# charles-cooper/Smoothed-Particle-Hydrodynamics

Hardware: AMD Instinct MI355X
Metric: particle-steps/sec (whole node) (higher is better)
Workload: dtype f32; 1 GPU; config4_16M_box; particles=16507704, particles_per_gpu=16507704, cell_ids=wide, parallelism=1 GPU

## Files before the change

smoothed-particle-hydrodynamics_amd/csrc/sph_neighbors.hip:

```cpp
#include <stdlib.h>
#include <string.h>

#include <mutex>

#include "sph_common.h"

__global__ __launch_bounds__(SPH_BLOCK) void k_clear_neighbors(int32_t* __restrict__ nbrId, float* __restrict__ nbrDist,
                                                                uint16_t* __restrict__ nbr16, size_t n4) {
  const size_t i = (size_t)blockIdx.x * SPH_BLOCK + threadIdx.x;
  if (i >= n4) return;
  reinterpret_cast<int4*>(nbrId)[i] = make_int4(-1, -1, -1, -1);
  reinterpret_cast<float4*>(nbrDist)[i] = make_float4(-1.f, -1.f, -1.f, -1.f);
  if (i < n4 / 2) reinterpret_cast<int4*>(nbr16)[i] = make_int4(-1, -1, -1, -1);
}

int sphk_clear_neighbors(sph_solver* s) {
  const size_t n4 = (size_t)((s->d.N + SPH_TILE - 1) / SPH_TILE) * 64 * 8;
  hipLaunchKernelGGL(k_clear_neighbors, dim3((unsigned)((n4 + SPH_BLOCK - 1) / SPH_BLOCK)), dim3(SPH_BLOCK), 0, s->stream,
                     s->d.nbrId, s->d.nbrDist, s->d.nbr16, n4);
  SPH_HIP(hipGetLastError());
  return SPH_OK;
}

struct FnParams {
  int G, gx, gy, rangeLo, rangeHi;
  int idxLo, idxHi;
  int gz, bandCap;
  float h, cellSize, cellSizeInv, simScale, xmin, ymin, zmin;
};
struct FnArrays {
  const float4* sortedPos;
  const uint32_t *keys, *cellStart;
  int32_t* nbrId;
  float* nbrDist;
  uint16_t* nbr16;
};

__device__ __forceinline__ int wrap_cell(int c, int G) {
  if (c < 0) c += G;
  if (c >= G) c -= G;
  return c;
}

#define FN_PART 128
#define FN_THREADS (2 * FN_PART)
#define FN_PER_WAVE 32
#define FN_WAVES (FN_THREADS / 64)
#define FN_CAND_CAP 4096
#define FN_STAGE_PER 8
#define FN_WIN 16
#define FN_CAND_PAD 16
#define FN_LIST_CAP 48
#define FN_CHUNK 8
#define FN_SLOTS_PER_LANE (SPH_MAXN / 2)

typedef float f32x2 __attribute__((ext_vector_type(2)));
typedef float f32x4 __attribute__((ext_vector_type(4)));

#define FN_DST_STRIDE 36
#define FN_STAGE_BYTES (FN_PER_WAVE * (FN_DST_STRIDE * 4 + SPH_MAXN * 2))
#define FN_LIST_ROWS ((FN_STAGE_BYTES + 127) / 128 > FN_LIST_CAP ? (FN_STAGE_BYTES + 127) / 128 : FN_LIST_CAP)

struct FnShared {
  float x[FN_CAND_CAP + FN_CAND_PAD], y[FN_CAND_CAP + FN_CAND_PAD], z[FN_CAND_CAP + FN_CAND_PAD];
  uint16_t list[FN_WAVES][FN_LIST_ROWS][64];
  float binU[64];
  int rowLo[9], rowHi[9], rowBase[9];
  int win[9][FN_WIN];
  int winTrue[9][FN_WIN];
  uint32_t hist[FN_WAVES][32];
#ifdef FN_STAMPS
  uint32_t stamps[16];
#endif
};
static_assert(FN_LIST_ROWS >= FN_LIST_CAP, "the wave's list area holds the lists first, the staging of the store phase afterwards");

__device__ __forceinline__ int pair_other(int v) { return __builtin_amdgcn_update_dpp(0, v, 0xB1, 0xf, 0xf, true); }
typedef unsigned long long fn_mask_t;
static_assert(FN_LIST_CAP <= 64, "one bit per list entry");

#ifdef FN_STAMPS
#define FN_STAMP(ph)                                                                                      \
  {                                                                                                       \
    const unsigned long long t_ = __builtin_amdgcn_s_memtime();                                           \
    if ((threadIdx.x & 63) == 0) atomicAdd(&sh.stamps[(ph)], (uint32_t)(t_ - stamp_));                    \
    stamp_ = __builtin_amdgcn_s_memtime();                                                                \
  }
#else
#define FN_STAMP(ph)
#endif

template <bool BANDS>
__device__ __forceinline__ void fn_exact_walk(const FnParams& d, const FnArrays& g, FnShared& sh, int id, int wave, int lane) {
  const float4 me = g.sortedPos[id];
  const int myCell = (int)g.keys[id];
  int lo[8], hi[8], ldsBase[8];
  {
    const float px = me.x - d.xmin, py = me.y - d.ymin, pz = me.z - d.zmin;
    const float cfx = (float)(int)(me.x * d.cellSizeInv) * d.cellSize;
    const float cfy = (float)(int)(me.y * d.cellSizeInv) * d.cellSize;
    const float cfz = (float)(int)(me.z * d.cellSizeInv) * d.cellSize;
    const int dx = ((px - cfx) < d.h) ? -1 : 1;
    const int dy = ((py - cfy) < d.h) ? -1 : 1;
    const int dz = ((pz - cfz) < d.h) ? -1 : 1;
    const int sy = dy * d.gx, sz = dz * d.gx * d.gy;
    const int off[8] = {0, dx, sy, sz, dx + sy, dx + sz, sy + sz, dx + sy + sz};
    const int ry = dy + 1, rz = dz + 1;
    const int rows[8] = {4, 4, ry + 3, 1 + 3 * rz, ry + 3, 1 + 3 * rz, ry + 3 * rz, ry + 3 * rz};
#pragma unroll
    for (int k = 0; k < 8; k++) {
      const int raw = myCell + off[k];
      int c = wrap_cell(raw, d.G);
      const int r = (c == raw && (!BANDS || rows[k] == 4)) ? rows[k] : -1;
      c = min(max(c, 0), d.G - 1);
      lo[k] = (int)g.cellStart[c];
      hi[k] = (int)g.cellStart[c + 1];
      if (hi[k] - lo[k] > (1 << 20)) hi[k] = lo[k];
      ldsBase[k] = -1;
      if (r >= 0 && hi[k] > lo[k] && lo[k] >= sh.rowLo[r] && hi[k] <= sh.rowHi[r]) ldsBase[k] = sh.rowBase[r] + (lo[k] - sh.rowLo[r]);
    }
  }
  if (lane < 32) sh.hist[wave][lane] = 0u;
  const unsigned long long ltMask = (lane == 0) ? 0ull : (~0ull >> (64 - lane));
  const float h2 = d.h * d.h;
#pragma unroll
  for (int k = 0; k < 8; k++) {
    for (int j0 = lo[k]; j0 < hi[k]; j0 += 64) {
      const int j = j0 + lane;
      if (j < hi[k] && j != id) {
        float ox, oy, oz;
        if (ldsBase[k] >= 0) { const int sl = ldsBase[k] + (j - lo[k]); ox = sh.x[sl]; oy = sh.y[sl]; oz = sh.z[sl]; }
        else { const float4 o = g.sortedPos[j]; ox = o.x; oy = o.y; oz = o.z; }
        const float ex = me.x - ox, ey = me.y - oy, ez = me.z - oz;
        const float d2 = ex * ex + ey * ey + ez * ez;
        if (d2 <= h2) {
          const float dist = sqrtf(d2);
          const int bin = (int)(dist * (float)SPH_RSEG / d.h);
          if (bin < SPH_RSEG) atomicAdd(&sh.hist[wave][bin], 1u);
        }
      }
    }
  }
  int jb = 0, sum = 0;
  while (jb < SPH_RSEG) {
    sum += (int)sh.hist[wave][jb];
    if (sum == SPH_MAXN) break;
    if (sum > SPH_MAXN) { jb--; break; }
    jb++;
  }
  const float r_thr = (float)(jb + 1) * d.h / (float)SPH_RSEG;
  const float r2 = r_thr * r_thr;
  int found = 0;
#pragma unroll
  for (int k = 0; k < 8; k++) {
    for (int j0 = lo[k]; j0 < hi[k] && found < SPH_MAXN; j0 += 64) {
      const int j = j0 + lane;
      float d2 = 0.f;
      bool hit = false;
      if (j < hi[k] && j != id) {
        float ox, oy, oz;
        if (ldsBase[k] >= 0) { const int sl = ldsBase[k] + (j - lo[k]); ox = sh.x[sl]; oy = sh.y[sl]; oz = sh.z[sl]; }
        else { const float4 o = g.sortedPos[j]; ox = o.x; oy = o.y; oz = o.z; }
        const float ex = me.x - ox, ey = me.y - oy, ez = me.z - oz;
        d2 = ex * ex + ey * ey + ez * ez;
        hit = d2 <= r2;
      }
      const unsigned long long m = __ballot(hit);
      const int pos = found + __popcll(m & ltMask);
      if (hit && pos < SPH_MAXN) {
        const size_t idx = nbr_index(id, pos);
        g.nbrId[idx] = j;
        g.nbrDist[idx] = sqrtf(d2) * d.simScale;
      }
      found += __popcll(m);
    }
  }
  if (lane >= min(found, SPH_MAXN) && lane < SPH_MAXN) {
    const size_t idx = nbr_index(id, lane);
    g.nbrId[idx] = -1;
    g.nbrDist[idx] = -1.f;
  }
  if (lane == 0) g.nbr16[nbr_index(id, 0)] = (uint16_t)SPH_N16_WIDE;
}

template <bool BANDS>
__global__ __launch_bounds__(FN_THREADS, 2) void k_find_neighbors(FnParams d, const float4* __restrict__ sortedPos,
                                                                   const uint32_t* __restrict__ keys,
                                                                   const uint32_t* __restrict__ cellStart,
                                                                   const float* __restrict__ binU, int32_t* __restrict__ nbrId,
                                                                   float* __restrict__ nbrDist, uint16_t* __restrict__ nbr16,
                                                                   int32_t* __restrict__ nbrBase, uint32_t* __restrict__ dbg,
                                                                   uint32_t* __restrict__ trace,
                                                                   const float4* __restrict__ bandPos,
                                                                   const uint32_t* __restrict__ bandStart) {
  extern __shared__ __align__(16) unsigned char fn_smem[];
  FnShared& sh = *reinterpret_cast<FnShared*>(fn_smem);
  const int tid = threadIdx.x, lane = tid & 63, wave = tid >> 6;
  const int p = tid >> 1, laneB = tid & 1;
  const int rangeBegin = max((int)cellStart[d.rangeLo], d.idxLo), rangeEnd = min((int)cellStart[d.rangeHi], d.idxHi);
  const int p0 = rangeBegin + blockIdx.x * FN_PART;
  if (p0 >= rangeEnd) return;
  const int id = p0 + p;
  const bool alive = id < rangeEnd;
  FnArrays g;
  g.sortedPos = sortedPos; g.keys = keys; g.cellStart = cellStart; g.nbrId = nbrId; g.nbrDist = nbrDist; g.nbr16 = nbr16;
#ifdef FN_STAMPS
  const unsigned long long wgStart_ = __builtin_amdgcn_s_memrealtime();
  if (tid < 16) sh.stamps[tid] = 0u;
  __syncthreads();
  unsigned long long stamp_ = __builtin_amdgcn_s_memtime();
#endif

  const int blockHi = min(p0 + FN_PART, rangeEnd);
  const float4 myPos = alive ? sortedPos[id] : make_float4(0.f, 0.f, 0.f, 0.f);
  const int myCell = alive ? (int)keys[id] : 0;
  int batchLo = p0, retry = 0;
  while (batchLo < blockHi) {
  int batchHi = blockHi;
  if (retry) {
    const unsigned row0 = keys[batchLo] / (unsigned)d.gx;
    int firstStop = FN_PART;
#pragma unroll
    for (int q = FN_PART / 64 - 1; q >= 0; q--) {
      const int iq = batchLo + 64 * q + lane;
      const bool stopq = (iq >= blockHi) || (keys[min(iq, blockHi - 1)] / (unsigned)d.gx != row0) || (retry == 2 && (q > 0 || lane >= 32));
      const unsigned long long mq = __ballot(stopq);
      if (mq) firstStop = 64 * q + __ffsll((long long)mq) - 1;
    }
    batchHi = min(batchLo + firstStop, blockHi);
  }
  const int cLo = (int)keys[batchLo], cHi = (int)keys[batchHi - 1];
  const int nc = cHi - cLo + 3;
  const bool winOk = nc + 1 <= FN_WIN;
  constexpr int order[9] = {4, 3, 5, 1, 7, 0, 2, 6, 8};
  int runLo[9], runN[9], total = 0;
  {
    const int q = min(lane >> 1, 8);
    const int r = (int)((0x862071534ull >> (4 * q)) & 15ull);
    const int shift = (r % 3 - 1) * d.gx + (r / 3 - 1) * d.gx * d.gy;
    const int cell = ((lane & 1) ? cHi + 2 : cLo - 1) + shift;
    const uint32_t* tbl = cellStart;
    if (BANDS && r != 4) tbl = bandStart + (size_t)(r - (r > 4 ? 1 : 0)) * ((size_t)d.G + 1);
    const int v = (int)tbl[min(max(cell, 0), d.G)];
#pragma unroll
    for (int qq = 0; qq < 9; qq++) {
      const int lo = __builtin_amdgcn_readlane(v, 2 * qq), hi = __builtin_amdgcn_readlane(v, 2 * qq + 1);
      runLo[qq] = lo; runN[qq] = max(hi - lo, 0);
      total += runN[qq];
    }
  }
  if (total > FN_CAND_CAP) {
    if (retry < 2) { retry++; continue; }
    total = 0;
#pragma unroll
    for (int q = 0; q < 9; q++) {
      if (total + runN[q] > FN_CAND_CAP) { runN[q] = 0; if (tid == 0) atomicAdd(&dbg[3], 1u); }
      total += runN[q];
    }
  }
  int se[9], sd[9];
  {
    int base = 0;
#pragma unroll
    for (int q = 0; q < 9; q++) { sd[q] = runLo[q] - base; base += runN[q]; se[q] = base; }
    if (BANDS) {
#pragma unroll
      for (int q = 1; q < 9; q++) sd[q] += (order[q] - (order[q] > 4 ? 1 : 0)) * d.bandCap;
    }
  }
  if (tid == 0) {
#pragma unroll
    for (int q = 0; q < 9; q++) { sh.rowLo[order[q]] = runLo[q]; sh.rowHi[order[q]] = runLo[q] + runN[q]; sh.rowBase[order[q]] = se[q] - runN[q]; }
  }
  if (winOk && tid < 9 * FN_WIN) {
    const int r = tid / FN_WIN, i = tid % FN_WIN;
    const int shift = (r % 3 - 1) * d.gx + (r / 3 - 1) * d.gx * d.gy;
    const int wc = min(max(cLo - 1 + shift + i, 0), d.G);
    if (BANDS) {
      const uint32_t* tbl = (r == 4) ? cellStart : bandStart + (size_t)(r - (r > 4 ? 1 : 0)) * ((size_t)d.G + 1);
      if (i <= nc) { sh.win[r][i] = (int)tbl[wc]; sh.winTrue[r][i] = (int)cellStart[wc]; }
    } else {
      if (i <= nc) sh.win[r][i] = (int)cellStart[wc];
    }
  }
  if (tid >= 192 && tid < 256) sh.binU[tid - 192] = binU[tid - 192];
  FN_STAMP(0)
  {
    constexpr int PER = FN_STAGE_PER;
#pragma unroll 1
    for (int f0 = 0; f0 < total; f0 += PER * FN_THREADS) {
      float4 rec[PER];
#pragma unroll
      for (int u = 0; u < PER; u++) {
        const int f = min(f0 + tid + u * FN_THREADS, total - 1);
        int delta = sd[0];
#pragma unroll
        for (int q = 0; q < 8; q++) delta = (f >= se[q]) ? sd[q + 1] : delta;
        if (BANDS) rec[u] = (f >= se[0] ? bandPos : sortedPos)[f + delta];
        else rec[u] = sortedPos[f + delta];
      }
#pragma unroll
      for (int u = 0; u < PER; u++) {
        const int f = f0 + tid + u * FN_THREADS;
        if (f < total) { sh.x[f] = rec[u].x; sh.y[f] = rec[u].y; sh.z[f] = rec[u].z; }
      }
    }
  }
  __syncthreads();
  FN_STAMP(3)
  const bool mine_now = alive && id >= batchLo && id < batchHi;
  bool slow = false;

  if (mine_now) {
  float4 me = myPos;
  int myCellNow = myCell, idNow = id;
  asm volatile("" : "+v"(me.x), "+v"(me.y), "+v"(me.z), "+v"(myCellNow), "+v"(idNow));
  int pLo[4], pHi[4], absDelta[4];
  int selfSlot = -1;
  int zLoMine = 0;
  int trueLo[4] = {0, 0, 0, 0}, trueHi[4] = {0, 0, 0, 0};
  {
    const float px = me.x - d.xmin, py = me.y - d.ymin, pz = me.z - d.zmin;
    const float cfx = (float)(int)(me.x * d.cellSizeInv) * d.cellSize;
    const float cfy = (float)(int)(me.y * d.cellSizeInv) * d.cellSize;
    const float cfz = (float)(int)(me.z * d.cellSizeInv) * d.cellSize;
    const int dx = ((px - cfx) < d.h) ? -1 : 1;
    const int dy = ((py - cfy) < d.h) ? -1 : 1;
    const int dz = ((pz - cfz) < d.h) ? -1 : 1;
    const int sy = dy * d.gx, sz = dz * d.gx * d.gy;
    const int ry = dy + 1, rz = dz + 1;
    const bool stepX[4] = {laneB != 0, laneB == 0, laneB == 0, laneB == 0};
    const bool stepY[4] = {false, true, false, true};
    const bool stepZ[4] = {false, false, true, true};
#pragma unroll
    for (int i = 0; i < 4; i++) {
      const int xs = stepX[i] ? dx : 0;
      const int raw = myCellNow + xs + (stepY[i] ? sy : 0) + (stepZ[i] ? sz : 0);
      const int row = (stepY[i] ? ry : 1) + 3 * (stepZ[i] ? rz : 1);
      const int c = wrap_cell(raw, d.G);
      int lo, hi;
      int tLo, tHi;
      const bool staged = c == raw;
      const bool banded = BANDS && i != 0;
      if (staged && winOk) {
        const int w = myCellNow - cLo + 1 + xs;
        lo = sh.win[row][w];
        hi = sh.win[row][w + 1];
        tLo = lo; tHi = hi;
        if (banded) { tLo = sh.winTrue[row][w]; tHi = sh.winTrue[row][w + 1]; }
      } else {
        const int cc = min(max(c, 0), d.G - 1);
        lo = tLo = (int)cellStart[cc];
        hi = tHi = (int)cellStart[cc + 1];
        if (banded && staged) {
          const uint32_t* tbl = bandStart + (size_t)(row - (row > 4 ? 1 : 0)) * ((size_t)d.G + 1);
          lo = (int)tbl[cc];
          hi = (int)tbl[cc + 1];
        }
      }
      const int n = hi - lo;
      int base = 0;
      if (n > 0) {
        if (staged && lo >= sh.rowLo[row] && hi <= sh.rowHi[row]) base = sh.rowBase[row] + (lo - sh.rowLo[row]);
        else slow = true;
      }
      pLo[i] = base;
      pHi[i] = base + n;
      absDelta[i] = lo - base;
      if (banded) absDelta[i] += (row - (row > 4 ? 1 : 0)) * d.bandCap;
      if (i == 2) zLoMine = tLo;
      if (i == 0 && laneB == 0) selfSlot = base + (idNow - lo);
      if (BANDS) { trueLo[i] = tLo; trueHi[i] = tHi; }
    }
    if (BANDS) {
      const int cx = (int)(me.x * d.cellSizeInv), cy = (int)(me.y * d.cellSizeInv), cz = (int)(me.z * d.cellSizeInv);
      const bool premise = me.x >= 0.f && me.y >= 0.f && me.z >= 0.f && me.x < 1.0e9f && me.y < 1.0e9f && me.z < 1.0e9f && cx < d.gx &&
                           cy < d.gy && cz < d.gz && myCellNow == cx + cy * d.gx + cz * d.gx * d.gy;
      if (!premise) slow = true;
    }
  }
  int wideB = 0;
  if (BANDS) {
    const int zOther = pair_other(zLoMine);
    const int zB = laneB ? zLoMine : zOther;
#pragma unroll
    for (int i = 0; i < 4; i++) {
      const bool zf = i >= 2;
      const int rel = SPH_N16_BIAS - (zf ? zB : idNow);
      if (trueHi[i] > trueLo[i] && (trueLo[i] + rel < 0 || trueHi[i] - 1 + rel > SPH_N16_MAX)) wideB = 1;
    }
  }
  {
    const int other = pair_other((int)slow);
    slow = slow || (other != 0);
  }
  if (slow) {
#pragma unroll
    for (int i = 0; i < 4; i++) pHi[i] = pLo[i];
    if (laneB == 0) atomicAdd(&dbg[0], 1u);
  }
  FN_STAMP(4)

  int cnt = 0;
  int segEnd[4];
  const f32x2 mx = {me.x, me.x}, my = {me.y, me.y}, mz = {me.z, me.z};
  const float r2f = sh.binU[63];
  const f32x2 nthr = {-r2f, -r2f};
  float neg1s = -1.f;
  asm volatile("" : "+s"(neg1s));
  const f32x2 neg1 = {neg1s, neg1s};
  uint16_t (*const myList)[64] = sh.list[wave];
#define FN_DIFF(m, c) __builtin_elementwise_fma((c), neg1, (m))
#define FN_TEST(X, Y, Z)                                                                        \
  {                                                                                             \
    const f32x2 ex0 = FN_DIFF(mx, X.xy), ex1 = FN_DIFF(mx, X.zw), ey0 = FN_DIFF(my, Y.xy), ey1 = FN_DIFF(my, Y.zw); \
    const f32x2 ez0 = FN_DIFF(mz, Z.xy), ez1 = FN_DIFF(mz, Z.zw);                               \
    const f32x2 s0 = __builtin_elementwise_fma(ez0, ez0, __builtin_elementwise_fma(ey0, ey0, __builtin_elementwise_fma(ex0, ex0, nthr))); \
    const f32x2 s1 = __builtin_elementwise_fma(ez1, ez1, __builtin_elementwise_fma(ey1, ey1, __builtin_elementwise_fma(ex1, ex1, nthr))); \
    acc = __builtin_amdgcn_alignbit(acc, __float_as_uint(s0.x), 31);                            \
    acc = __builtin_amdgcn_alignbit(acc, __float_as_uint(s0.y), 31);                            \
    acc = __builtin_amdgcn_alignbit(acc, __float_as_uint(s1.x), 31);                            \
    acc = __builtin_amdgcn_alignbit(acc, __float_as_uint(s1.y), 31);                            \
  }
#define FN_FLUSH(k)                                                                             \
  {                                                                                             \
    uint32_t m = ((k) == 0) ? 0u : (acc << (32 - (k)));          \
    const int lowT = pieceLo - aBase, hiT = pieceHi - aBase;                                    \
    if (lowT > 0) m &= 0xffffffffu >> lowT;                \
    if (hiT < 32) m &= ~(0xffffffffu >> hiT);                         \
    if (i == 0) {                                                      \
      const unsigned ts = (unsigned)(selfSlot - aBase);                                         \
      if (ts < 32u) m &= ~(0x80000000u >> ts);                                                  \
    }                                                                                           \
    cnt += __popc(m);                                                                           \
    if (cnt > FN_LIST_CAP) m = 0u;                         \
    while (m != 0u) {                                                                           \
      const int bpos = __clz((int)m);                                                           \
      *wr = (uint16_t)(aBase + bpos);                                                           \
      wr += 64;                                                    \
      m &= ~(0x80000000u >> bpos);                                                              \
    }                                                                                           \
  }
  uint16_t* wr = &myList[0][lane];
#pragma unroll
  for (int i = 0; i < 4; i++) {
    const int pieceLo = pLo[i], pieceHi = pHi[i];
    if (pieceHi > pieceLo) {
      int a = pieceLo & ~3;
      int aBase = a, k = 0;
      uint32_t acc = 0u;
      f32x4 X = *reinterpret_cast<const f32x4*>(&sh.x[a]);
      f32x4 Y = *reinterpret_cast<const f32x4*>(&sh.y[a]);
      f32x4 Z = *reinterpret_cast<const f32x4*>(&sh.z[a]);
      f32x4 Xb = *reinterpret_cast<const f32x4*>(&sh.x[a + 4]);
      f32x4 Yb = *reinterpret_cast<const f32x4*>(&sh.y[a + 4]);
      f32x4 Zb = *reinterpret_cast<const f32x4*>(&sh.z[a + 4]);
      while (a < pieceHi) {
        FN_TEST(X, Y, Z)
        X = *reinterpret_cast<const f32x4*>(&sh.x[a + 8]);
        Y = *reinterpret_cast<const f32x4*>(&sh.y[a + 8]);
        Z = *reinterpret_cast<const f32x4*>(&sh.z[a + 8]);
        __builtin_amdgcn_sched_barrier(0);
        FN_TEST(Xb, Yb, Zb)
        Xb = *reinterpret_cast<const f32x4*>(&sh.x[a + 12]);
        Yb = *reinterpret_cast<const f32x4*>(&sh.y[a + 12]);
        Zb = *reinterpret_cast<const f32x4*>(&sh.z[a + 12]);
        __builtin_amdgcn_sched_barrier(0);
        a += 8; k += 8;
        if (k == 32) { FN_FLUSH(32) aBase = a; k = 0; }
      }
      FN_FLUSH(k)
    }
    segEnd[i] = cnt;
  }
#undef FN_TEST
#undef FN_FLUSH
  FN_STAMP(5)
  int over = cnt > FN_LIST_CAP ? 1 : 0;
  over |= pair_other(over);
  if (over) {
    if (laneB == 0 && !slow) atomicAdd(&dbg[1], 1u);
    slow = true;
#pragma unroll
    for (int i = 0; i < 4; i++) segEnd[i] = 0;
  }

  const int total = segEnd[3];
  float d2v[FN_LIST_CAP];
  uint32_t slotPk[FN_LIST_CAP / 2];
  int idxv[FN_LIST_CAP];
#pragma unroll
  for (int c0 = 0; c0 < FN_LIST_CAP; c0 += FN_CHUNK) {
    if (__any(c0 < total)) {
      int slotv[FN_CHUNK];
#pragma unroll
      for (int u = 0; u < FN_CHUNK; u++) slotv[u] = min((int)myList[c0 + u][lane], FN_CAND_CAP + FN_CAND_PAD - 1);
      if (BANDS) {
#pragma unroll
        for (int u = 0; u < FN_CHUNK; u++) {
          const int e = c0 + u;
          int dlt = absDelta[1];
          dlt = (e >= segEnd[1]) ? absDelta[2] : dlt;
          dlt = (e >= segEnd[2]) ? absDelta[3] : dlt;
          int v = slotv[u] + absDelta[0];
          if (e >= segEnd[0] && e < total) v = __float_as_int(bandPos[slotv[u] + dlt].w);
          idxv[e] = v;
        }
      }
#pragma unroll
      for (int u = 0; u < FN_CHUNK; u++) {
        const int sl = slotv[u];
        const float ex = me.x - sh.x[sl], ey = me.y - sh.y[sl], ez = me.z - sh.z[sl];
        const float v = ex * ex + ey * ey + ez * ez;
        d2v[c0 + u] = (c0 + u < total) ? v : __builtin_inff();
      }
      if (!BANDS) {
#pragma unroll
        for (int u = 0; u < FN_CHUNK; u += 2) slotPk[(c0 + u) >> 1] = (uint32_t)slotv[u] | ((uint32_t)slotv[u + 1] << 16);
      }
    } else {
#pragma unroll
      for (int u = 0; u < FN_CHUNK; u++) d2v[c0 + u] = __builtin_inff();
      if (BANDS) {
#pragma unroll
        for (int u = 0; u < FN_CHUNK; u++) idxv[c0 + u] = 0;
      } else {
#pragma unroll
        for (int u = 0; u < FN_CHUNK; u += 2) slotPk[(c0 + u) >> 1] = 0u;
      }
    }
  }
  FN_STAMP(6)
  int liveEnd = FN_CHUNK;
#pragma unroll
  for (int c0 = FN_CHUNK; c0 < FN_LIST_CAP; c0 += FN_CHUNK) liveEnd = __any(c0 < total) ? c0 + FN_CHUNK : liveEnd;
  int lo = 0, hi = SPH_RSEG, cAtHi = 0;
#pragma unroll 1
  for (int it = 0; it < 5; it++) {
    const int mid = (lo + hi) >> 1;
    const float U = sh.binU[min(mid, SPH_RSEG - 1)];
    int c = 0;
#pragma unroll
    for (int c0 = 0; c0 < FN_LIST_CAP; c0 += FN_CHUNK) {
      if (c0 < liveEnd) {
#pragma unroll
        for (int u = 0; u < FN_CHUNK; u++) c += (d2v[c0 + u] < U) ? 1 : 0;
      }
    }
    c += pair_other(c);
    if (lo < hi) {
      if (c >= SPH_MAXN) { hi = mid; cAtHi = c; } else lo = mid + 1;
    }
  }
  const int jb = (lo >= SPH_RSEG) ? SPH_RSEG : ((cAtHi == SPH_MAXN) ? lo : lo - 1);
  const float r2 = sh.binU[32 + jb];
  FN_STAMP(7)

  fn_mask_t acc = 0;
#pragma unroll
  for (int c0 = 0; c0 < FN_LIST_CAP; c0 += FN_CHUNK) {
    if (c0 < liveEnd) {
#pragma unroll
      for (int u = 0; u < FN_CHUNK; u++) acc |= (d2v[c0 + u] <= r2) ? ((fn_mask_t)1 << (c0 + u)) : (fn_mask_t)0;
    }
  }
  fn_mask_t below[4];
#pragma unroll
  for (int i = 0; i < 4; i++) below[i] = (segEnd[i] >= (int)(8 * sizeof(fn_mask_t))) ? ~(fn_mask_t)0 : (((fn_mask_t)1 << segEnd[i]) - 1);
  int mine[4];
  mine[0] = __popcll(acc & below[0]);
#pragma unroll
  for (int i = 1; i < 4; i++) mine[i] = __popcll(acc & below[i] & ~below[i - 1]);
  const int cellTot = mine[0] | (mine[1] << 8) | (mine[2] << 16) | (mine[3] << 24);
  const int otherTot = pair_other(cellTot);
  const int zLoOther = pair_other(zLoMine);
  if (!slow) {
    const int c0b = cellTot & 255, c1b = (cellTot >> 8) & 255, c2b = (cellTot >> 16) & 255, c3b = (cellTot >> 24) & 255;
    const int o0b = otherTot & 255, o1b = (otherTot >> 8) & 255, o2b = (otherTot >> 16) & 255, o3b = (otherTot >> 24) & 255;
    const int run = min(c0b + c1b + c2b + c3b + o0b + o1b + o2b + o3b, SPH_MAXN);
    const int front = c0b + o0b + (laneB ? c1b + c2b : o1b + o2b);
    int start[4];
    start[0] = laneB ? o0b : 0;
    start[1] = laneB ? o0b + c0b : front;
    start[2] = laneB ? o0b + c0b + c1b : front + c1b;
    start[3] = laneB ? front + o1b + o2b : front + c1b + c2b + o3b;
    const int zBase = laneB ? zLoMine : zLoOther;
    int rel16[4];
    int wide = 0;
#pragma unroll
    for (int i = 0; i < 4; i++) {
      const bool zf = i >= 2;
      rel16[i] = absDelta[i] - (zf ? zBase : idNow) + SPH_N16_BIAS;
      if (pHi[i] > pLo[i] && (pLo[i] + rel16[i] < 0 || pHi[i] - 1 + rel16[i] > SPH_N16_MAX)) wide = 1;
    }
    if (BANDS) wide = wideB;
    int own16 = SPH_N16_BIAS - idNow, far16 = SPH_N16_BIAS + 0x8000 - zBase;
    asm volatile("" : "+v"(own16), "+v"(far16));
    wide |= pair_other(wide);
    int tidNow = tid;
    asm volatile("" : "+v"(tidNow));
    float* const waveArea = reinterpret_cast<float*>(&sh.list[0][0][0]) + (tidNow >> 6) * (FN_LIST_ROWS * 64 / 2);
    float* const dstRow = waveArea + ((tidNow & 63) >> 1) * FN_DST_STRIDE;
    uint16_t* const idRow = reinterpret_cast<uint16_t*>(waveArea + FN_PER_WAVE * FN_DST_STRIDE) + ((tidNow & 63) >> 1) * SPH_MAXN;
#pragma unroll
    for (int v = 0; v < FN_SLOTS_PER_LANE / 8; v++)
      *reinterpret_cast<uint4*>(idRow + FN_SLOTS_PER_LANE * laneB + 8 * v) = make_uint4(0xffffffffu, 0xffffffffu, 0xffffffffu, 0xffffffffu);
    const uint32_t mapBase = ((uint32_t)(idNow >> 6) * (8u * 64u) + (uint32_t)(idNow & 63)) << 2;
    int curStart = start[0], curDelta = absDelta[0], rank = 0;
#pragma unroll
    for (int c0 = 0; c0 < FN_LIST_CAP; c0 += FN_CHUNK) {
      if (!__any(c0 < total)) continue;
#pragma unroll
      for (int u = 0; u < FN_CHUNK; u++) {
        const int e = c0 + u;
        if (e == segEnd[0]) { curStart = start[1]; curDelta = absDelta[1]; rank = 0; }
        if (e == segEnd[1]) { curStart = start[2]; curDelta = absDelta[2]; rank = 0; }
        if (e == segEnd[2]) { curStart = start[3]; curDelta = absDelta[3]; rank = 0; }
        if ((acc >> e) & 1) {
          const int pos = curStart + rank;
          rank++;
          if (pos < SPH_MAXN) {
            const int jn = BANDS ? idxv[e] : (int)((slotPk[e >> 1] >> ((e & 1) * 16)) & 0xffffu) + curDelta;
            const int o16 = jn + own16;
            idRow[pos] = (uint16_t)((uint32_t)o16 <= (uint32_t)SPH_N16_MAX ? o16 : jn + far16);
            dstRow[pos] = d2v[e];
          }
        }
      }
    }
    if (__any(wide != 0)) {
    int curStart = start[0], curDelta = absDelta[0], rank = 0;
#pragma unroll
    for (int c0 = 0; c0 < FN_LIST_CAP; c0 += FN_CHUNK) {
      if (!__any(c0 < total)) continue;
#pragma unroll
      for (int u = 0; u < FN_CHUNK; u++) {
        const int e = c0 + u;
        if (e == segEnd[0]) { curStart = start[1]; curDelta = absDelta[1]; rank = 0; }
        if (e == segEnd[1]) { curStart = start[2]; curDelta = absDelta[2]; rank = 0; }
        if (e == segEnd[2]) { curStart = start[3]; curDelta = absDelta[3]; rank = 0; }
        if ((acc >> e) & 1) {
          const int pos = curStart + rank;
          rank++;
          if (pos < SPH_MAXN) {
            const int jn = BANDS ? idxv[e] : (int)((slotPk[e >> 1] >> ((e & 1) * 16)) & 0xffffu) + curDelta;
            if (wide) nbrId[mapBase + (uint32_t)(((pos >> 2) << 8) + (pos & 3))] = jn;
          }
        }
      }
    }
    }
    if (wide) {
      for (int k = run + laneB; k < SPH_MAXN; k += 2) nbrId[mapBase + (uint32_t)(((k >> 2) << 8) + (k & 3))] = -1;
    }
    if (laneB == 0) nbrBase[idNow] = zBase;
    const uint32_t mapMine = mapBase + (uint32_t)((FN_SLOTS_PER_LANE / 4) * laneB) * 256u;
#pragma unroll
    for (int v = 0; v < FN_SLOTS_PER_LANE / 8; v++) {
      const uint4 q = *reinterpret_cast<const uint4*>(idRow + FN_SLOTS_PER_LANE * laneB + 8 * v);
      *reinterpret_cast<uint2*>(nbr16 + (size_t)(mapMine + (uint32_t)(2 * v) * 256u)) = make_uint2(q.x, q.y);
      *reinterpret_cast<uint2*>(nbr16 + (size_t)(mapMine + (uint32_t)(2 * v + 1) * 256u)) = make_uint2(q.z, q.w);
    }
    if (wide && laneB == 0) {
      nbr16[mapBase] = (uint16_t)SPH_N16_WIDE;
      atomicAdd(&dbg[2], 1u);
    }
#pragma unroll
    for (int gq = 0; gq < FN_SLOTS_PER_LANE / 4; gq++) {
      const f32x4 dq = *reinterpret_cast<const f32x4*>(dstRow + FN_SLOTS_PER_LANE * laneB + 4 * gq);
      const float dv[4] = {dq.x, dq.y, dq.z, dq.w};
      float out[4];
#pragma unroll
      for (int j = 0; j < 4; j++) out[j] = (FN_SLOTS_PER_LANE * laneB + 4 * gq + j < run) ? sqrtf(dv[j]) * d.simScale : -1.f;
      *reinterpret_cast<f32x4*>(nbrDist + (size_t)(mapMine + (uint32_t)gq * 256u)) = f32x4{out[0], out[1], out[2], out[3]};
    }
  }
  FN_STAMP(8)
  }

  {
    unsigned long long todo = __ballot(mine_now && slow && laneB == 0);
    while (todo != 0ull) {
      const int b = __ffsll((long long)todo) - 1;
      todo &= todo - 1ull;
      fn_exact_walk<BANDS>(d, g, sh, p0 + wave * FN_PER_WAVE + (b >> 1), wave, lane);
    }
  }
  FN_STAMP(9)
  batchLo = batchHi;
  if (batchLo < blockHi) __syncthreads();
  }
#ifdef FN_STAMPS
  __syncthreads();
  if (tid < 16) atomicAdd(&dbg[16 + tid], sh.stamps[tid] >> 6);
  if (tid == 0) {
    const size_t row = 4 * ((size_t)(d.idxLo / FN_PART) + blockIdx.x);
    trace[row + 0] = (uint32_t)wgStart_;
    trace[row + 1] = (uint32_t)__builtin_amdgcn_s_memrealtime();
    trace[row + 2] = __builtin_amdgcn_s_getreg((31 << 11) | 4);
    trace[row + 3] = __builtin_amdgcn_s_getreg((31 << 11) | 20);
  }
#endif
}

int sphk_find_neighbors(sph_solver* s, int ghostDepth, int idxLo, int idxHi, hipStream_t stream, bool bands) {
  if (idxLo < 0 || idxLo % SPH_BLOCK != 0) { sph_set_error("sphk_find_neighbors: idxLo %d is not a multiple of %d", idxLo, SPH_BLOCK); return SPH_ERR_INVALID; }
  if (bands && !s->bandBuf.p) { sph_set_error("sphk_find_neighbors: no search bands were built"); return SPH_ERR_ORDER; }
  idxHi = min(idxHi, s->d.N);
  if (idxHi <= idxLo) return SPH_OK;
  {
    static std::mutex mu;
    static bool attrSet[64] = {};
    std::lock_guard<std::mutex> lock(mu);
    const int dev = s->cfg.device;
    if (dev < 0 || dev >= 64 || !attrSet[dev]) {
      SPH_HIP(hipFuncSetAttribute((const void*)k_find_neighbors<false>, hipFuncAttributeMaxDynamicSharedMemorySize, (int)sizeof(FnShared)));
      SPH_HIP(hipFuncSetAttribute((const void*)k_find_neighbors<true>, hipFuncAttributeMaxDynamicSharedMemorySize, (int)sizeof(FnShared)));
      if (dev >= 0 && dev < 64) attrSet[dev] = true;
    }
  }
  const SphDev r = sph_ranged(s, ghostDepth);
  FnParams a;
  a.G = r.G; a.gx = r.gx; a.gy = r.gy; a.rangeLo = r.rangeLo; a.rangeHi = r.rangeHi;
  a.idxLo = idxLo; a.idxHi = idxHi;
  a.gz = r.gz; a.bandCap = s->capacity;
  a.h = r.h; a.cellSize = r.cellSize; a.cellSizeInv = r.cellSizeInv; a.simScale = r.simScale;
  a.xmin = r.xmin; a.ymin = r.ymin; a.zmin = r.zmin;
  SphBands b = {};
  if (bands) sphk_bands_bytes(s, &b);
  hipLaunchKernelGGL(bands ? k_find_neighbors<true> : k_find_neighbors<false>, dim3(sph_blocks(idxHi - idxLo, FN_PART)), dim3(FN_THREADS),
                     sizeof(FnShared), stream ? stream : s->stream, a,
                     (const float4*)r.sortedPos, (const uint32_t*)r.keys, (const uint32_t*)r.cellStart, r.binU, r.nbrId, r.nbrDist, r.nbr16,
                     r.nbrBase, r.dbg,
                     r.valsAlt , (const float4*)b.pos, (const uint32_t*)b.start);
  SPH_HIP(hipGetLastError());
  return SPH_OK;
}
```

Baseline: 1.442 billion particle-steps/s.

## Process two particle halves per block in banded neighbor search to reuse staged candidates

In the banded variant of the neighbor search kernel, each block now covers 256 particles instead of 128, using the same thread count. It stages one shared candidate window and loops twice over two halves of particles against it. If the combined window exceeds the candidate cap, it first falls back to per-half batches before the existing retry path. The goal is to amortize the cost of loading candidate positions into shared memory across more particles. The trade-off is fewer blocks, which means less parallelism, plus longer serial work per block and some extra registers.

```diff
diff --git a/smoothed-particle-hydrodynamics_amd/csrc/sph_neighbors.hip b/smoothed-particle-hydrodynamics_amd/csrc/sph_neighbors.hip
--- a/smoothed-particle-hydrodynamics_amd/csrc/sph_neighbors.hip
+++ b/smoothed-particle-hydrodynamics_amd/csrc/sph_neighbors.hip
@@ -42,8 +42,10 @@
   return c;
 }
 
-#define FN_PART 128
-#define FN_THREADS (2 * FN_PART)
+#define FN_HALF 128
+#define FN_THREADS (2 * FN_HALF)
+#define FN_PART(BANDS) ((BANDS) ? 2 * FN_HALF : FN_HALF)
+static_assert(SPH_CHUNK_ALIGN % FN_PART(true) == 0 && SPH_CHUNK_ALIGN % FN_PART(false) == 0, "tiles stay whole inside chunk launches");
 #define FN_PER_WAVE 32
 #define FN_WAVES (FN_THREADS / 64)
 #define FN_CAND_CAP 4096
@@ -198,7 +200,8 @@
   const int tid = threadIdx.x, lane = tid & 63, wave = tid >> 6;
   const int p = tid >> 1, laneB = tid & 1;
   const int rangeBegin = max((int)cellStart[d.rangeLo], d.idxLo), rangeEnd = min((int)cellStart[d.rangeHi], d.idxHi);
-  const int p0 = rangeBegin + blockIdx.x * FN_PART;
+  constexpr int PART = FN_PART(BANDS), HALVES = PART / FN_HALF;
+  const int p0 = rangeBegin + blockIdx.x * PART;
   if (p0 >= rangeEnd) return;
   const int id = p0 + p;
   const bool alive = id < rangeEnd;
@@ -211,17 +214,25 @@
   unsigned long long stamp_ = __builtin_amdgcn_s_memtime();
 #endif
 
-  const int blockHi = min(p0 + FN_PART, rangeEnd);
-  const float4 myPos = alive ? sortedPos[id] : make_float4(0.f, 0.f, 0.f, 0.f);
-  const int myCell = alive ? (int)keys[id] : 0;
+  const int blockHi = min(p0 + PART, rangeEnd);
+  float4 myPos[HALVES];
+  int myCell[HALVES];
+#pragma unroll
+  for (int hf = 0; hf < HALVES; hf++) {
+    const bool aliveH = hf ? id + hf * FN_HALF < rangeEnd : alive;
+    myPos[hf] = aliveH ? sortedPos[id + hf * FN_HALF] : make_float4(0.f, 0.f, 0.f, 0.f);
+    myCell[hf] = aliveH ? (int)keys[id + hf * FN_HALF] : 0;
+  }
   int batchLo = p0, retry = 0;
+  bool halves = false;
   while (batchLo < blockHi) {
   int batchHi = blockHi;
+  if (HALVES > 1 && halves && !retry) batchHi = min(p0 + ((batchLo - p0) / FN_HALF + 1) * FN_HALF, blockHi);
   if (retry) {
     const unsigned row0 = keys[batchLo] / (unsigned)d.gx;
-    int firstStop = FN_PART;
-#pragma unroll
-    for (int q = FN_PART / 64 - 1; q >= 0; q--) {
+    int firstStop = FN_HALF;
+#pragma unroll
+    for (int q = FN_HALF / 64 - 1; q >= 0; q--) {
       const int iq = batchLo + 64 * q + lane;
       const bool stopq = (iq >= blockHi) || (keys[min(iq, blockHi - 1)] / (unsigned)d.gx != row0) || (retry == 2 && (q > 0 || lane >= 32));
       const unsigned long long mq = __ballot(stopq);
@@ -250,6 +261,7 @@
     }
   }
   if (total > FN_CAND_CAP) {
+    if (HALVES > 1 && !halves) { halves = true; continue; }
     if (retry < 2) { retry++; continue; }
     total = 0;
 #pragma unroll
@@ -308,12 +320,18 @@
   }
   __syncthreads();
   FN_STAMP(3)
-  const bool mine_now = alive && id >= batchLo && id < batchHi;
+  int hf = 0;
+#pragma unroll 1
+  do {
+  const int idH = id + hf * FN_HALF;
+  const bool mine_now = (hf ? idH < rangeEnd : alive) && idH >= batchLo && idH < batchHi;
+  if (HALVES > 1 && !__any(mine_now)) continue;
   bool slow = false;
 
   if (mine_now) {
-  float4 me = myPos;
-  int myCellNow = myCell, idNow = id;
+  float4 me = myPos[0];
+  int myCellNow = myCell[0], idNow = idH;
+  if (HALVES > 1 && hf) { me = myPos[HALVES - 1]; myCellNow = myCell[HALVES - 1]; }
   asm volatile("" : "+v"(me.x), "+v"(me.y), "+v"(me.z), "+v"(myCellNow), "+v"(idNow));
   int pLo[4], pHi[4], absDelta[4];
   int selfSlot = -1;
@@ -683,10 +701,11 @@
     while (todo != 0ull) {
       const int b = __ffsll((long long)todo) - 1;
       todo &= todo - 1ull;
-      fn_exact_walk<BANDS>(d, g, sh, p0 + wave * FN_PER_WAVE + (b >> 1), wave, lane);
+      fn_exact_walk<BANDS>(d, g, sh, p0 + hf * FN_HALF + wave * FN_PER_WAVE + (b >> 1), wave, lane);
     }
   }
   FN_STAMP(9)
+  } while (HALVES > 1 && ++hf < HALVES);
   batchLo = batchHi;
   if (batchLo < blockHi) __syncthreads();
   }
@@ -694,7 +713,7 @@
   __syncthreads();
   if (tid < 16) atomicAdd(&dbg[16 + tid], sh.stamps[tid] >> 6);
   if (tid == 0) {
-    const size_t row = 4 * ((size_t)(d.idxLo / FN_PART) + blockIdx.x);
+    const size_t row = 4 * ((size_t)(d.idxLo / PART) + blockIdx.x);
     trace[row + 0] = (uint32_t)wgStart_;
     trace[row + 1] = (uint32_t)__builtin_amdgcn_s_memrealtime();
     trace[row + 2] = __builtin_amdgcn_s_getreg((31 << 11) | 4);
@@ -728,7 +747,8 @@
   a.xmin = r.xmin; a.ymin = r.ymin; a.zmin = r.zmin;
   SphBands b = {};
   if (bands) sphk_bands_bytes(s, &b);
-  hipLaunchKernelGGL(bands ? k_find_neighbors<true> : k_find_neighbors<false>, dim3(sph_blocks(idxHi - idxLo, FN_PART)), dim3(FN_THREADS),
+  hipLaunchKernelGGL(bands ? k_find_neighbors<true> : k_find_neighbors<false>,
+                     dim3(sph_blocks(idxHi - idxLo, bands ? FN_PART(true) : FN_PART(false))), dim3(FN_THREADS),
                      sizeof(FnShared), stream ? stream : s->stream, a,
                      (const float4*)r.sortedPos, (const uint32_t*)r.keys, (const uint32_t*)r.cellStart, r.binU, r.nbrId, r.nbrDist, r.nbr16,
                      r.nbrBase, r.dbg,
```

Result: faster. 1.470 billion particle-steps/s, median of 6 (+2.0%).
